# Anttwo/MACARONS

Hardware: AMD Instinct MI355X
Metric: candidate-camera coverage-gain evals/sec (100k pts, 200 cams) (higher is better)
Workload: dtype f32; 1 GPU; scorer: B=1 cloud x N=100000 points x C=200 cameras per GPU (BASELINE headline 100k pts / 200 cams), inputs resident in HBM; points=100000, cams_per_gpu=200, parallelism=camera-shard x1, streams=2

## Files before the change

macarons_amd/csrc/local_pct7.hip:

```cpp
#ifdef L7_TRACE
#define LP_TRACE L7_TRACE
#endif
#include "lp_tile.h"

namespace mcr {
namespace v7 {

using namespace tile;

#ifndef L7_PF
#define L7_PF 3
#endif
constexpr int PF = L7_PF;
__device__ __forceinline__ float l7_gelu(float x) {
    const float w = fabsf(x) * 0.84932180028801904f;
    const float t = __builtin_amdgcn_rcpf(fmaf(w, 0.39169198f, 1.0f));
    float q = fmaf(0.7478556f, t, -0.0958798f);
    q = fmaf(q, t, 0.3480242f);
    q *= t;
    const float e = __builtin_amdgcn_exp2f(-(w * w));
    const float erfa = fmaf(-q, e, 1.0f);
    const float hx = 0.5f * x;
    return fmaf(fabsf(hx), erfa, hx);
}

constexpr int PR = 17;
struct WRing { uint4 b[PF]; };

__device__ __forceinline__ const uint4* wptr(const float* Wp, int nt, int S, int lane) {
    return reinterpret_cast<const uint4*>(Wp) + (size_t)nt * S * 64 + lane;
}
template <int S>
__device__ __forceinline__ void wload(WRing& r, const uint4* bp) {
#pragma unroll
    for (int p = 0; p < (S < PF ? S : PF); ++p) {
        r.b[p] = bp[p * 64];
    }
    __builtin_amdgcn_sched_barrier(0);
}

__device__ __forceinline__ void fetch(uint4 (&an)[2], const uint4* __restrict__ A, int s, int i, int h) {
    const int c = 2 * s + h;
#pragma unroll
    for (int mt = 0; mt < 2; ++mt) an[mt] = A[(mt * 32 + i) * PR + c];
}

template <int S, class Fn>
__device__ __forceinline__ void gemm_with(f32x16 (&acc)[2], const uint4* __restrict__ A, WRing& r, const uint4* __restrict__ bp,
                                          int lane_, Fn fn) {
    const int lane = opaque(lane_);
    const int i = lane & 31, h = lane >> 5;
    uint4 an[2];
    fetch(an, A, 0, i, h);
#pragma unroll
    for (int s = 0; s < S; ++s) {
        const uint4 a0 = an[0], a1 = an[1];
        if (s + 1 < S) fetch(an, A, s + 1, i, h);
        const uint4 w = r.b[s % PF];
        if (s + PF < S) r.b[s % PF] = bp[(s + PF) * 64];
        __builtin_amdgcn_sched_barrier(0);
        acc[0] = mfma_h(w, a0, acc[0]);
        acc[1] = mfma_h(w, a1, acc[1]);
        fn(s);
        pin(acc[0], acc[1]);
        __builtin_amdgcn_sched_barrier(0);
    }
}
template <int S>
__device__ __forceinline__ void gemm(f32x16 (&acc)[2], const uint4* __restrict__ A, WRing& r, const uint4* __restrict__ bp,
                                     int lane_) {
    gemm_with<S>(acc, A, r, bp, lane_, [](int) {});
}

__device__ __forceinline__ void gemm_qkv(f32x16 (&acc)[2], f32x16& acch, const uint4* __restrict__ A, WRing& r0, WRing& r1,
                                         const uint4* __restrict__ bp0, const uint4* __restrict__ bp1, int wave, int lane_) {
    constexpr int S = 8;
    const int lane = opaque(lane_);
    const int i = lane & 31, h = lane >> 5, mh = wave & 1;
    uint4 an[2];
    fetch(an, A, 0, i, h);
#pragma unroll
    for (int s = 0; s < S; ++s) {
        const uint4 a0 = an[0], a1 = an[1];
        const uint4 ah = mh ? a1 : a0;
        if (s + 1 < S) fetch(an, A, s + 1, i, h);
        const uint4 w = r0.b[s % PF], v = r1.b[s % PF];
        if (s + PF < S) {
            r0.b[s % PF] = bp0[(s + PF) * 64];
            r1.b[s % PF] = bp1[(s + PF) * 64];
        }
        __builtin_amdgcn_sched_barrier(0);
        acc[0] = mfma_h(w, a0, acc[0]);
        acc[1] = mfma_h(w, a1, acc[1]);
        acch = mfma_h(v, ah, acch);
        pin(acc[0], acc[1], acch);
        __builtin_amdgcn_sched_barrier(0);
    }
}

__device__ __forceinline__ void add_bias(f32x16& x, const float* __restrict__ vec, int nt, int lane_) {
    const float4* p = reinterpret_cast<const float4*>(vec + 32 * nt + 4 * (opaque(lane_) >> 5));
#pragma unroll
    for (int g = 0; g < 4; ++g) {
        const float4 b = p[2 * g];
        x[4 * g] += b.x; x[4 * g + 1] += b.y; x[4 * g + 2] += b.z; x[4 * g + 3] += b.w;
    }
}

__device__ __forceinline__ void put4(uint2* __restrict__ plane, int idx, float v0, float v1, float v2, float v3) {
    plane[idx] = make_uint2(pack2h(v0, v1), pack2h(v2, v3));
}
template <class Fn>
__device__ __forceinline__ void put_planes(uint4* __restrict__ buf, int nt, int mt, const f32x16& t, int lane_, Fn f) {
    const int lane = opaque(lane_);
    const int j = lane & 31, h = lane >> 5;
    uint2* b2 = reinterpret_cast<uint2*>(buf) + (mt * 32 + j) * (2 * PR) + h + 8 * nt;
#pragma unroll
    for (int g = 0; g < 4; ++g) {
        put4(b2, 2 * g, f(t[4 * g], g, 0), f(t[4 * g + 1], g, 1), f(t[4 * g + 2], g, 2), f(t[4 * g + 3], g, 3));
        __builtin_amdgcn_sched_barrier(0);
    }
}
template <class Fn>
__device__ __forceinline__ void put_quad(uint4* __restrict__ buf, int nt, int mt, int g, const f32x16& t, int row, Fn f) {
    uint2* b2 = reinterpret_cast<uint2*>(buf);
    put4(b2, mt * (32 * 2 * PR) + row + 2 * (4 * nt + g), f(t[4 * g]), f(t[4 * g + 1]), f(t[4 * g + 2]), f(t[4 * g + 3]));
}
template <class Fn>
__device__ __forceinline__ void put_f32(float* __restrict__ buf, int LD, int kmask, int chunk0, int mt, const f32x16& t, int lane_, Fn f) {
    const int lane = opaque(lane_);
    const int j = lane & 31, h = lane >> 5, key = j & kmask;
    float* row = buf + (mt * 32 + j) * LD;
#pragma unroll
    for (int g = 0; g < 4; ++g)
        *reinterpret_cast<float4*>(row + (((chunk0 + 2 * g + h) ^ key) << 2)) =
            make_float4(f(t[4 * g], g, 0), f(t[4 * g + 1], g, 1), f(t[4 * g + 2], g, 2), f(t[4 * g + 3], g, 3));
}

__device__ __forceinline__ void ln_partial(const f32x16 (&x)[2], float2* __restrict__ St, int wave, int lane_) {
    const int lane = opaque(lane_);
#pragma unroll
    for (int mt = 0; mt < 2; ++mt) {
#ifdef L7_LN_TWO_PASS
        float s = 0.f;
#pragma unroll
        for (int r = 0; r < 16; r += 4) s += (x[mt][r] + x[mt][r + 1]) + (x[mt][r + 2] + x[mt][r + 3]);
        const float m = halves_sum(s) * (1.0f / 32.f);
        float q = 0.f;
#pragma unroll
        for (int r = 0; r < 16; ++r) {
            const float d = x[mt][r] - m;
            q = fmaf(d, d, q);
        }
        q = halves_sum(q);
        St[wave * 64 + mt * 32 + (lane & 31)] = make_float2(m, q);
#else
        float s = 0.f, q = 0.f;
#pragma unroll
        for (int r = 0; r < 16; r += 4) s += (x[mt][r] + x[mt][r + 1]) + (x[mt][r + 2] + x[mt][r + 3]);
#pragma unroll
        for (int r = 0; r < 16; ++r) q = fmaf(x[mt][r], x[mt][r], q);
        s = halves_sum(s);
        q = halves_sum(q);
        const float m = s * (1.0f / 32.f);
        St[wave * 64 + mt * 32 + (lane & 31)] = make_float2(m, fmaxf(fmaf(-s, m, q), 0.f));
#endif
    }
}
__device__ __forceinline__ void ln_finish(const f32x16 (&x)[2], const float2* __restrict__ St, uint4* __restrict__ P, int wave,
                                          int lane_) {
    const int j = opaque(lane_) & 31;
#pragma unroll
    for (int mt = 0; mt < 2; ++mt) {
        float2 p[4];
#pragma unroll
        for (int w = 0; w < 4; ++w) p[w] = St[w * 64 + mt * 32 + j];
        const float mu = ((p[0].x + p[1].x) + (p[2].x + p[3].x)) * 0.25f;
        float m2 = (p[0].y + p[1].y) + (p[2].y + p[3].y), dd = 0.f;
#pragma unroll
        for (int w = 0; w < 4; ++w) {
            const float d = p[w].x - mu;
            dd = fmaf(d, d, dd);
        }
        m2 = fmaf(32.f, dd, m2);
        const float rstd = __builtin_amdgcn_rsqf(fmaf(m2, 1.0f / 128.f, 1e-5f));
        const float shift = -mu * rstd;
        put_planes(P, wave, mt, x[mt], lane_, [&](float v, int, int) { return fmaf(v, rstd, shift); });
    }
}

#ifndef L7_WGS
#define L7_WGS 3
#endif
__global__ __launch_bounds__(256, L7_WGS) void local_pct7_kernel(const float* __restrict__ offs, float* __restrict__ feat,
                                                                long long ld_feat, long long S,
                                                                const float* __restrict__ blob, _Float16* __restrict__ feat_h) {
    __shared__ __attribute__((aligned(16))) uint4 P[64 * PR];
    __shared__ __attribute__((aligned(16))) uint4 H[2 * 64 * 16];
    __shared__ __attribute__((aligned(16))) float2 St[4 * 64];
    __shared__ __attribute__((aligned(16))) uint4 Z[4];
    float* F = reinterpret_cast<float*>(H);
    const int tid = threadIdx.x, lane0 = tid & 63;
    const int wave = __builtin_amdgcn_readfirstlane(tid >> 6);
    if (tid < 4) Z[tid] = make_uint4(0, 0, 0, 0);
    const float* mats = blob;
    const float* vecs = blob + L7_MATS_TOTAL;
    const long long s0 = (long long)blockIdx.x * L3_QPB;
    const int lane = lane0;
    int tp = 0; (void)tp;
    LP_T();
    WRing ring;
    f32x16 acc[2], xres[2];
    wload<1>(ring, wptr(mats + l7_mat_off(0), wave, 1, lane));
    init_bias(acc[0], vecs + LP_VEC_EMB1, wave, lane);
    init_bias(acc[1], vecs + LP_VEC_EMB1, wave, lane);
    float xyz[2][3];
    {
        const int j = lane & 31;
#pragma unroll
        for (int mt = 0; mt < 2; ++mt) {
            const int t = mt * 32 + j;
            const long long seq = s0 + (t >> 4);
            xyz[mt][0] = xyz[mt][1] = xyz[mt][2] = 0.f;
            if (seq < S) {
                const float* p = offs + (seq * 16 + (t & 15)) * 3;
                xyz[mt][0] = p[0]; xyz[mt][1] = p[1]; xyz[mt][2] = p[2];
            }
        }
        const bool lowh = lane < 32;
#pragma unroll
        for (int mt = 0; mt < 2; ++mt) {
            uint4 a = make_uint4(0, 0, 0, 0);
            a.x = pack2h(lowh ? xyz[mt][0] : 0.f, lowh ? xyz[mt][1] : 0.f);
            a.y = pack2h(lowh ? xyz[mt][2] : 0.f, 0.f);
            acc[mt] = mfma_h(ring.b[0], a, acc[mt]);
        }
    }
    LP_T();
    wload<8>(ring, wptr(mats + l7_mat_off(1), wave, 8, lane));
#pragma unroll
    for (int mt = 0; mt < 2; ++mt)
        put_planes(H, wave, mt, acc[mt], lane, [&](float v, int, int) { return l7_gelu(v); });
    init_bias(xres[0], vecs + LP_VEC_EMB2, wave, lane);
    init_bias(xres[1], vecs + LP_VEC_EMB2, wave, lane);
    __syncthreads();
    LP_T();
    gemm<8>(xres, H, ring, wptr(mats + l7_mat_off(1), wave, 8, lane), lane);
    LP_T();
    {
        const bool cat = wave == 3 && lane >= 32;
#pragma unroll
        for (int mt = 0; mt < 2; ++mt) {
            xres[mt][13] = cat ? xyz[mt][0] : xres[mt][13];
            xres[mt][14] = cat ? xyz[mt][1] : xres[mt][14];
            xres[mt][15] = cat ? xyz[mt][2] : xres[mt][15];
        }
    }

#pragma unroll 1
    for (int e = 0; e < 2; ++e) {
        const float* em = mats + l7_mat_off(2) + e * (L7_MAT_QKV + 5 * L7_MAT_128);
        const float* ev = vecs + LP_VEC_ENC0 + e * LP_VEC_ENC_STRIDE;
        const float* w_out = em + L7_MAT_QKV;
        const float* w_ff1a = w_out + L7_MAT_128;
        const float* w_ff1b = w_out + L7_MAT_128 * 2;
        const float* w_ff2a = w_out + L7_MAT_128 * 3;
        const float* w_ff2b = w_out + L7_MAT_128 * 4;
        WRing ring1;
        const uint4* bq0 = wptr(em, wave, 8, lane);
        const uint4* bq1 = wptr(em, 4 + (wave >> 1), 8, lane);
        wload<8>(ring, bq0);
        wload<8>(ring1, bq1);
        LP_T();
        ln_partial(xres, St, wave, lane);
        __syncthreads();
        LP_T();
        ln_finish(xres, St, P, wave, lane);
        __syncthreads();
        LP_T();
        {
            f32x16 aq[2], ah;
            const int nth = 4 + (wave >> 1);
            init_bias(aq[0], ev, wave, lane);
            init_bias(aq[1], ev, wave, lane);
            init_bias(ah, ev, nth, lane);
            gemm_qkv(aq, ah, P, ring, ring1, bq0, bq1, wave, lane);
            LP_T();
            wload<8>(ring, wptr(w_out, wave, 8, lane));
            __syncthreads();
            LP_T();
            auto fb = [&](float v, int, int) { return v; };
            uint4* dst = wave < 2 ? P : H;
            const int ntd = wave < 2 ? wave : wave - 2;
#pragma unroll
            for (int mt = 0; mt < 2; ++mt) put_planes(dst, ntd, mt, aq[mt], lane, fb);
            put_planes(H, nth - 2, wave & 1, ah, lane, fb);
        }
        __syncthreads();
        LP_T();
        {
            typedef _Float16 h16x4 __attribute__((ext_vector_type(4)));
            typedef short s16x4 __attribute__((ext_vector_type(4)));
            typedef __attribute__((address_space(3))) s16x4 lds_s16x4;
            const int ln = opaque(lane);
            const int r0 = wave * 16, li = ln & 15, g = ln >> 4;
            const char* Pb = reinterpret_cast<const char*>(P);
            const char* ka = Pb + (r0 + li) * (16 * PR) + 64 + (g & 1) * 8;
            const char* qa = g < 2 ? Pb + (r0 + li) * (16 * PR) + g * 8 : reinterpret_cast<const char*>(Z);
            const char* va = reinterpret_cast<const char*>(H) + (r0 + 4 * g + (li >> 2)) * (16 * PR) + (li & 3) * 8;
            h16x4 pf[4];
#pragma unroll
            for (int hh = 0; hh < 4; ++hh) {
                const h16x4 kf = *reinterpret_cast<const h16x4*>(ka + 16 * hh);
                const h16x4 qf = *reinterpret_cast<const h16x4*>(qa + 16 * hh);
                f32x4 st = __builtin_amdgcn_mfma_f32_16x16x16f16(kf, qf, f32x4{0.f, 0.f, 0.f, 0.f}, 0, 0, 0);
                float mx = fmaxf(fmaxf(st[0], st[1]), fmaxf(st[2], st[3]));
                mx = rows_allreduce(mx, [](float a, float b) { return fmaxf(a, b); });
                mx *= 0.35355339059327376220f;
                float den = 0.f;
#pragma unroll
                for (int r = 0; r < 4; ++r) {
                    st[r] = __expf(fmaf(st[r], 0.35355339059327376220f, -mx));
                    den += st[r];
                }
                den = rows_allreduce(den, [](float a, float b) { return a + b; });
                const float inv = __builtin_amdgcn_rcpf(den);
                const uint2 pk = make_uint2(pack2h(st[0] * inv, st[1] * inv), pack2h(st[2] * inv, st[3] * inv));
                pf[hh] = __builtin_bit_cast(h16x4, pk);
            }
            f32x4 o[4][2];
#pragma unroll
            for (int hh = 0; hh < 4; ++hh)
#pragma unroll
                for (int nt = 0; nt < 2; ++nt) {
                    const s16x4 vt = __builtin_amdgcn_ds_read_tr16_b64_v4i16((lds_s16x4*)(va + 64 * hh + 32 * nt));
                    o[hh][nt] = __builtin_amdgcn_mfma_f32_16x16x16f16(__builtin_bit_cast(h16x4, vt), pf[hh], f32x4{0.f, 0.f, 0.f, 0.f}, 0, 0, 0);
                }
            asm volatile("s_waitcnt lgkmcnt(0)" ::: "memory");
            uint2* p2 = reinterpret_cast<uint2*>(P);
            const int base = (r0 + li) * (2 * PR) + g;
#pragma unroll
            for (int hh = 0; hh < 4; ++hh)
#pragma unroll
                for (int nt = 0; nt < 2; ++nt)
                    put4(p2, base + 2 * (4 * hh + 2 * nt), o[hh][nt][0], o[hh][nt][1], o[hh][nt][2], o[hh][nt][3]);
        }
        LP_T();
        add_bias(xres[0], ev + 192, wave, lane);
        add_bias(xres[1], ev + 192, wave, lane);
        __syncthreads();
        LP_T();
        gemm<8>(xres, P, ring, wptr(w_out, wave, 8, lane), lane);
        LP_T();
        wload<8>(ring, wptr(w_ff1a, wave, 8, lane));
        ln_partial(xres, St, wave, lane);
        init_bias(acc[0], ev + 192 + 128, wave, lane);
        init_bias(acc[1], ev + 192 + 128, wave, lane);
        __syncthreads();
        LP_T();
        ln_finish(xres, St, P, wave, lane);
        __syncthreads();
        LP_T();
        gemm<8>(acc, P, ring, wptr(w_ff1a, wave, 8, lane), lane);
        LP_T();
        wload<8>(ring, wptr(w_ff1b, wave, 8, lane));
        f32x16 accb[2];
        init_bias(accb[0], ev + 192 + 128 + 128, wave, lane);
        init_bias(accb[1], ev + 192 + 128 + 128, wave, lane);
        const int pq_lane = opaque(lane), pq_row = (pq_lane & 31) * (2 * PR) + (pq_lane >> 5);
        gemm_with<8>(accb, P, ring, wptr(w_ff1b, wave, 8, lane), lane, [&](int s_) {
            put_quad(H, wave, s_ >> 2, s_ & 3, acc[s_ >> 2], pq_row, [&](float v) { return l7_gelu(v); });
        });
        LP_T();
        wload<8>(ring, wptr(w_ff2a, wave, 8, lane));
        add_bias(xres[0], ev + 192 + 128 + 256, wave, lane);
        add_bias(xres[1], ev + 192 + 128 + 256, wave, lane);
        __syncthreads();
        LP_T();
        gemm_with<8>(xres, H, ring, wptr(w_ff2a, wave, 8, lane), lane, [&](int s_) {
            put_quad(P, wave, s_ >> 2, s_ & 3, accb[s_ >> 2], pq_row, [&](float v) { return l7_gelu(v); });
        });
        LP_T();
        wload<8>(ring, wptr(w_ff2b, wave, 8, lane));
        __syncthreads();
        LP_T();
        LP_T();
        gemm<8>(xres, P, ring, wptr(w_ff2b, wave, 8, lane), lane);
        LP_T();
    }
    LP_T();
    wload<8>(ring, wptr(mats + l7_mat_off(14), wave, 8, lane));
    ln_partial(xres, St, wave, lane);
    init_bias(acc[0], vecs + LP_VEC_LIN0, wave, lane);
    init_bias(acc[1], vecs + LP_VEC_LIN0, wave, lane);
    __syncthreads();
    ln_finish(xres, St, P, wave, lane);
    __syncthreads();
    gemm<8>(acc, P, ring, wptr(mats + l7_mat_off(14), wave, 8, lane), lane);
#pragma unroll
    for (int mt = 0; mt < 2; ++mt)
        put_f32(F, 128, 15, 8 * wave, mt, acc[mt], lane, [&](float v, int, int) { return v; });
    __syncthreads();
    LP_T();
#pragma unroll
    for (int r = 0; r < 2; ++r) {
        const int o = tid + r * 256, q = o >> 7, c = o & 127;
        if (s0 + q < S) {
            float mx = -__builtin_inff(), sm = 0.f;
#pragma unroll
            for (int j = 0; j < 16; ++j) {
                const int row = q * 16 + j;
                const float v = F[row * 128 + ((((c >> 2) ^ (row & 15)) << 2) | (c & 3))];
                mx = fmaxf(mx, v);
                sm += v;
            }
            const float av = sm * (1.0f / 16.f);
            if (feat_h) {
                const unsigned hv = pack2h(mx, av);
                const long long o2 = (s0 + q) * ld_feat + c;
                feat_h[o2] = __builtin_bit_cast(_Float16, (unsigned short)(hv & 0xffffu));
                feat_h[o2 + 128] = __builtin_bit_cast(_Float16, (unsigned short)(hv >> 16));
            } else {
                feat[(s0 + q) * ld_feat + c] = mx;
                feat[(s0 + q) * ld_feat + 128 + c] = av;
            }
        }
    }
    LP_T();
}

}

void launch_local_pct7(hipStream_t s, const float* offs, float* feat, int64_t ld_feat, int64_t S, const float* blob, void* feat_h) {
    if (S <= 0) return;
    hipLaunchKernelGGL(v7::local_pct7_kernel, dim3((unsigned)cdiv(S, L3_QPB)), dim3(256), 0, s, offs, feat, (long long)ld_feat,
                       (long long)S, blob, (_Float16*)feat_h);
}

int local_pct7_blob_floats() { return L7_BLOB_FLOATS; }

}
```

Baseline: 4.777 million evals/s.

## Use logistic-form GELU fit, packed f16 mix FMAs, and precomputed lane byte offsets

Replaces the erf-polynomial GELU with a fitted logistic form x/(1+exp2(x*p(x^2))), using constants generated by a new minimax-fit script. LayerNorm normalisation and softmax scaling now write f16 pairs directly through v_fma_mix instructions, and the softmax uses exp2 with the log2(e) factor folded into the scale. Per-lane address components (weight, bias, fragment row, plane row, stats) are computed once into a Lane struct as byte offsets, which removes repeated index arithmetic and opaque() calls. The goal is fewer VALU instructions in the per-point MLP/attention kernel, at the cost of a slightly different GELU approximation error.

```diff
diff --git a/macarons_amd/csrc/gelu7_consts.inc b/macarons_amd/csrc/gelu7_consts.inc
--- /dev/null
+++ b/macarons_amd/csrc/gelu7_consts.inc
@@ -0,0 +1,4 @@
+constexpr float GELU7_K1 = -2.30112134f;
+constexpr float GELU7_K3 = -0.106775724f;
+constexpr float GELU7_K5 = 0.00101426308f;
+constexpr float GELU7_U0 = 64.0f;
diff --git a/macarons_amd/csrc/gen_gelu7_consts.py b/macarons_amd/csrc/gen_gelu7_consts.py
--- /dev/null
+++ b/macarons_amd/csrc/gen_gelu7_consts.py
@@ -0,0 +1,78 @@
+#!/usr/bin/env python3
+import math
+
+import numpy as np
+
+X = np.arange(-9000, 9001) * 1e-3
+PHI = np.array([0.5 * math.erfc(-x / math.sqrt(2.0)) for x in X])
+GELU = X * PHI
+U = X * X
+
+
+def max_err(c):
+    z = -X * (c[0] + U * (c[1] + U * c[2]))
+    with np.errstate(over="ignore"):
+        return float(np.max(np.abs(X / (1.0 + np.exp(z)) - GELU)))
+
+
+def nelder_mead(f, x0, step, iters=4000):
+    n = len(x0)
+    pts = [np.array(x0, dtype=np.float64)] + [np.array(x0, dtype=np.float64) + step[i] * np.eye(n)[i] for i in range(n)]
+    val = [f(p) for p in pts]
+    for _ in range(iters):
+        order = np.argsort(val)
+        pts, val = [pts[i] for i in order], [val[i] for i in order]
+        cen = np.mean(pts[:-1], axis=0)
+        refl = cen + (cen - pts[-1])
+        fr = f(refl)
+        if fr < val[0]:
+            ex = cen + 2.0 * (cen - pts[-1])
+            fe = f(ex)
+            pts[-1], val[-1] = (ex, fe) if fe < fr else (refl, fr)
+        elif fr < val[-2]:
+            pts[-1], val[-1] = refl, fr
+        else:
+            con = cen + 0.5 * (pts[-1] - cen)
+            fc = f(con)
+            if fc < val[-1]:
+                pts[-1], val[-1] = con, fc
+            else:
+                pts = [pts[0]] + [pts[0] + 0.5 * (p - pts[0]) for p in pts[1:]]
+                val = [val[0]] + [f(p) for p in pts[1:]]
+    k = int(np.argmin(val))
+    return pts[k], val[k]
+
+
+def fit():
+    sel = (X > 0) & (X <= 5.0)
+    x, ph = X[sel], PHI[sel]
+    y = np.log(ph / (1.0 - ph)) / x
+    A = np.stack([np.ones_like(x), x * x, x ** 4], axis=1)
+    c = np.linalg.lstsq(A, y, rcond=None)[0]
+    best = max_err(c)
+    for _ in range(12):
+        c2, e2 = nelder_mead(max_err, c, [1e-3 * abs(v) for v in c])
+        if e2 >= best * (1.0 - 1e-6):
+            break
+        c, best = c2, e2
+    return c, best
+
+
+def main():
+    c, err = fit()
+    u_star = -c[1] / (2.0 * c[2])
+    U0 = 64.0
+    p_u0 = c[0] + U0 * (c[1] + U0 * c[2])
+    assert c[2] < 0 and u_star < U0 and p_u0 > 1.0, (c, u_star, p_u0)
+    k = [-v / math.log(2.0) for v in c]
+    print("// Generated by gen_gelu7_consts.py -- do not edit.  Logistic-form erf GELU: x / (1 + exp(-x (c1 + c3 u + c5 u^2))), u = min(x^2, U0).")
+    print(f"// minimax fit on [-9, 9]: c = ({c[0]:.9g}, {c[1]:.9g}, {c[2]:.9g}), max |error| on the GELU {err:.3g} (double precision);")
+    print(f"// the polynomial peaks at u = {u_star:.4g} < U0; p(U0) = {p_u0:.4g}.  K = -log2(e) c: the exponent of v_exp_f32 directly.")
+    print(f"constexpr float GELU7_K1 = {k[0]:.9g}f;")
+    print(f"constexpr float GELU7_K3 = {k[1]:.9g}f;")
+    print(f"constexpr float GELU7_K5 = {k[2]:.9g}f;")
+    print(f"constexpr float GELU7_U0 = {U0:.1f}f;")
+
+
+if __name__ == "__main__":
+    main()
diff --git a/macarons_amd/csrc/local_pct7.hip b/macarons_amd/csrc/local_pct7.hip
--- a/macarons_amd/csrc/local_pct7.hip
+++ b/macarons_amd/csrc/local_pct7.hip
@@ -12,52 +12,73 @@
 #define L7_PF 3
 #endif
 constexpr int PF = L7_PF;
-__device__ __forceinline__ float l7_gelu(float x) {
-    const float w = fabsf(x) * 0.84932180028801904f;
-    const float t = __builtin_amdgcn_rcpf(fmaf(w, 0.39169198f, 1.0f));
-    float q = fmaf(0.7478556f, t, -0.0958798f);
-    q = fmaf(q, t, 0.3480242f);
-    q *= t;
-    const float e = __builtin_amdgcn_exp2f(-(w * w));
-    const float erfa = fmaf(-q, e, 1.0f);
-    const float hx = 0.5f * x;
-    return fmaf(fabsf(hx), erfa, hx);
-}
+#include "gelu7_consts.inc"
+__device__ __forceinline__ float l7_gate(float x) {
+    const float u = fminf(x * x, GELU7_U0);
+    float p = fmaf(u, GELU7_K5, GELU7_K3);
+    p = fmaf(p, u, GELU7_K1);
+    const float e = __builtin_amdgcn_exp2f(p * x);
+    return __builtin_amdgcn_rcpf(1.0f + e);
+}
+__device__ __forceinline__ unsigned fma2h(float a0, float b0, float c0, float a1, float b1, float c1) {
+    unsigned d;
+    asm("v_fma_mixlo_f16 %0, %1, %2, %3" : "=v"(d) : "v"(a0), "v"(b0), "v"(c0));
+    asm("v_fma_mixhi_f16 %0, %1, %2, %3" : "+v"(d) : "v"(a1), "v"(b1), "v"(c1));
+    return d;
+}
+__device__ __forceinline__ unsigned mul2h(float a0, float b0, float a1, float b1) {
+    unsigned d;
+    const float nz = -0.0f;
+    asm("v_fma_mixlo_f16 %0, %1, %2, %3" : "=v"(d) : "v"(a0), "v"(b0), "s"(nz));
+    asm("v_fma_mixhi_f16 %0, %1, %2, %3" : "+v"(d) : "v"(a1), "v"(b1), "s"(nz));
+    return d;
+}
+__device__ __forceinline__ unsigned gelu2h(float a, float b) { return mul2h(a, l7_gate(a), b, l7_gate(b)); }
 
 constexpr int PR = 17;
+constexpr int ROWB = 16 * PR;
 struct WRing { uint4 b[PF]; };
 
-__device__ __forceinline__ const uint4* wptr(const float* Wp, int nt, int S, int lane) {
-    return reinterpret_cast<const uint4*>(Wp) + (size_t)nt * S * 64 + lane;
+struct Lane {
+    unsigned w16;
+    unsigned b16;
+    unsigned frow;
+    unsigned prow;
+    unsigned st8;
+};
+
+__device__ __forceinline__ const char* wptr(const float* Wp, int nt, int S) {
+    return reinterpret_cast<const char*>(Wp) + (unsigned)(nt * S) * 1024u;
+}
+__device__ __forceinline__ uint4 wstep(const char* bp, int s, unsigned w16) {
+    return *reinterpret_cast<const uint4*>(bp + s * 1024 + w16);
 }
 template <int S>
-__device__ __forceinline__ void wload(WRing& r, const uint4* bp) {
+__device__ __forceinline__ void wload(WRing& r, const char* bp, unsigned w16) {
 #pragma unroll
     for (int p = 0; p < (S < PF ? S : PF); ++p) {
-        r.b[p] = bp[p * 64];
+        r.b[p] = wstep(bp, p, w16);
     }
     __builtin_amdgcn_sched_barrier(0);
 }
 
-__device__ __forceinline__ void fetch(uint4 (&an)[2], const uint4* __restrict__ A, int s, int i, int h) {
-    const int c = 2 * s + h;
-#pragma unroll
-    for (int mt = 0; mt < 2; ++mt) an[mt] = A[(mt * 32 + i) * PR + c];
+__device__ __forceinline__ void fetch(uint4 (&an)[2], const uint4* __restrict__ A, int s, unsigned frow) {
+    const char* a = reinterpret_cast<const char*>(A) + frow;
+#pragma unroll
+    for (int mt = 0; mt < 2; ++mt) an[mt] = *reinterpret_cast<const uint4*>(a + mt * 32 * ROWB + s * 32);
 }
 
 template <int S, class Fn>
-__device__ __forceinline__ void gemm_with(f32x16 (&acc)[2], const uint4* __restrict__ A, WRing& r, const uint4* __restrict__ bp,
-                                          int lane_, Fn fn) {
-    const int lane = opaque(lane_);
-    const int i = lane & 31, h = lane >> 5;
+__device__ __forceinline__ void gemm_with(f32x16 (&acc)[2], const uint4* __restrict__ A, WRing& r, const char* __restrict__ bp,
+                                          const Lane& L, Fn fn) {
     uint4 an[2];
-    fetch(an, A, 0, i, h);
+    fetch(an, A, 0, L.frow);
 #pragma unroll
     for (int s = 0; s < S; ++s) {
         const uint4 a0 = an[0], a1 = an[1];
-        if (s + 1 < S) fetch(an, A, s + 1, i, h);
+        if (s + 1 < S) fetch(an, A, s + 1, L.frow);
         const uint4 w = r.b[s % PF];
-        if (s + PF < S) r.b[s % PF] = bp[(s + PF) * 64];
+        if (s + PF < S) r.b[s % PF] = wstep(bp, s + PF, L.w16);
         __builtin_amdgcn_sched_barrier(0);
         acc[0] = mfma_h(w, a0, acc[0]);
         acc[1] = mfma_h(w, a1, acc[1]);
@@ -67,27 +88,26 @@
     }
 }
 template <int S>
-__device__ __forceinline__ void gemm(f32x16 (&acc)[2], const uint4* __restrict__ A, WRing& r, const uint4* __restrict__ bp,
-                                     int lane_) {
-    gemm_with<S>(acc, A, r, bp, lane_, [](int) {});
+__device__ __forceinline__ void gemm(f32x16 (&acc)[2], const uint4* __restrict__ A, WRing& r, const char* __restrict__ bp,
+                                     const Lane& L) {
+    gemm_with<S>(acc, A, r, bp, L, [](int) {});
 }
 
 __device__ __forceinline__ void gemm_qkv(f32x16 (&acc)[2], f32x16& acch, const uint4* __restrict__ A, WRing& r0, WRing& r1,
-                                         const uint4* __restrict__ bp0, const uint4* __restrict__ bp1, int wave, int lane_) {
+                                         const char* __restrict__ bp0, const char* __restrict__ bp1, int wave, const Lane& L) {
     constexpr int S = 8;
-    const int lane = opaque(lane_);
-    const int i = lane & 31, h = lane >> 5, mh = wave & 1;
+    const int mh = wave & 1;
     uint4 an[2];
-    fetch(an, A, 0, i, h);
+    fetch(an, A, 0, L.frow);
 #pragma unroll
     for (int s = 0; s < S; ++s) {
         const uint4 a0 = an[0], a1 = an[1];
         const uint4 ah = mh ? a1 : a0;
-        if (s + 1 < S) fetch(an, A, s + 1, i, h);
+        if (s + 1 < S) fetch(an, A, s + 1, L.frow);
         const uint4 w = r0.b[s % PF], v = r1.b[s % PF];
         if (s + PF < S) {
-            r0.b[s % PF] = bp0[(s + PF) * 64];
-            r1.b[s % PF] = bp1[(s + PF) * 64];
+            r0.b[s % PF] = wstep(bp0, s + PF, L.w16);
+            r1.b[s % PF] = wstep(bp1, s + PF, L.w16);
         }
         __builtin_amdgcn_sched_barrier(0);
         acc[0] = mfma_h(w, a0, acc[0]);
@@ -98,11 +118,20 @@
     }
 }
 
-__device__ __forceinline__ void add_bias(f32x16& x, const float* __restrict__ vec, int nt, int lane_) {
-    const float4* p = reinterpret_cast<const float4*>(vec + 32 * nt + 4 * (opaque(lane_) >> 5));
+__device__ __forceinline__ float4 bias4(const float* __restrict__ vec, int g, unsigned b16) {
+    return *reinterpret_cast<const float4*>(reinterpret_cast<const char*>(vec) + 32 * g + b16);
+}
+__device__ __forceinline__ void set_bias(f32x16& a, const float* __restrict__ vec, unsigned b16) {
 #pragma unroll
     for (int g = 0; g < 4; ++g) {
-        const float4 b = p[2 * g];
+        const float4 b = bias4(vec, g, b16);
+        a[4 * g] = b.x; a[4 * g + 1] = b.y; a[4 * g + 2] = b.z; a[4 * g + 3] = b.w;
+    }
+}
+__device__ __forceinline__ void add_bias(f32x16& x, const float* __restrict__ vec, unsigned b16) {
+#pragma unroll
+    for (int g = 0; g < 4; ++g) {
+        const float4 b = bias4(vec, g, b16);
         x[4 * g] += b.x; x[4 * g + 1] += b.y; x[4 * g + 2] += b.z; x[4 * g + 3] += b.w;
     }
 }
@@ -110,21 +139,18 @@
 __device__ __forceinline__ void put4(uint2* __restrict__ plane, int idx, float v0, float v1, float v2, float v3) {
     plane[idx] = make_uint2(pack2h(v0, v1), pack2h(v2, v3));
 }
-template <class Fn>
-__device__ __forceinline__ void put_planes(uint4* __restrict__ buf, int nt, int mt, const f32x16& t, int lane_, Fn f) {
-    const int lane = opaque(lane_);
-    const int j = lane & 31, h = lane >> 5;
-    uint2* b2 = reinterpret_cast<uint2*>(buf) + (mt * 32 + j) * (2 * PR) + h + 8 * nt;
+template <class Fn2>
+__device__ __forceinline__ void put_quad(uint4* __restrict__ buf, int mt, int g, const f32x16& t, unsigned row, Fn2 f2) {
+    *reinterpret_cast<uint2*>(reinterpret_cast<char*>(buf) + row + mt * 32 * ROWB + g * 16) =
+        make_uint2(f2(t[4 * g], t[4 * g + 1]), f2(t[4 * g + 2], t[4 * g + 3]));
+}
+template <class Fn2>
+__device__ __forceinline__ void put_planes(uint4* __restrict__ buf, int mt, const f32x16& t, unsigned row, Fn2 f2) {
 #pragma unroll
     for (int g = 0; g < 4; ++g) {
-        put4(b2, 2 * g, f(t[4 * g], g, 0), f(t[4 * g + 1], g, 1), f(t[4 * g + 2], g, 2), f(t[4 * g + 3], g, 3));
+        put_quad(buf, mt, g, t, row, f2);
         __builtin_amdgcn_sched_barrier(0);
     }
-}
-template <class Fn>
-__device__ __forceinline__ void put_quad(uint4* __restrict__ buf, int nt, int mt, int g, const f32x16& t, int row, Fn f) {
-    uint2* b2 = reinterpret_cast<uint2*>(buf);
-    put4(b2, mt * (32 * 2 * PR) + row + 2 * (4 * nt + g), f(t[4 * g]), f(t[4 * g + 1]), f(t[4 * g + 2]), f(t[4 * g + 3]));
 }
 template <class Fn>
 __device__ __forceinline__ void put_f32(float* __restrict__ buf, int LD, int kmask, int chunk0, int mt, const f32x16& t, int lane_, Fn f) {
@@ -137,8 +163,8 @@
             make_float4(f(t[4 * g], g, 0), f(t[4 * g + 1], g, 1), f(t[4 * g + 2], g, 2), f(t[4 * g + 3], g, 3));
 }
 
-__device__ __forceinline__ void ln_partial(const f32x16 (&x)[2], float2* __restrict__ St, int wave, int lane_) {
-    const int lane = opaque(lane_);
+__device__ __forceinline__ void ln_partial(const f32x16 (&x)[2], float2* __restrict__ St, int wave, const Lane& L) {
+    char* stw = reinterpret_cast<char*>(St + wave * 64) + L.st8;
 #pragma unroll
     for (int mt = 0; mt < 2; ++mt) {
 #ifdef L7_LN_TWO_PASS
@@ -153,7 +179,7 @@
             q = fmaf(d, d, q);
         }
         q = halves_sum(q);
-        St[wave * 64 + mt * 32 + (lane & 31)] = make_float2(m, q);
+        *reinterpret_cast<float2*>(stw + mt * 256) = make_float2(m, q);
 #else
         float s = 0.f, q = 0.f;
 #pragma unroll
@@ -163,18 +189,17 @@
         s = halves_sum(s);
         q = halves_sum(q);
         const float m = s * (1.0f / 32.f);
-        St[wave * 64 + mt * 32 + (lane & 31)] = make_float2(m, fmaxf(fmaf(-s, m, q), 0.f));
+        *reinterpret_cast<float2*>(stw + mt * 256) = make_float2(m, fmaxf(fmaf(-s, m, q), 0.f));
 #endif
     }
 }
-__device__ __forceinline__ void ln_finish(const f32x16 (&x)[2], const float2* __restrict__ St, uint4* __restrict__ P, int wave,
-                                          int lane_) {
-    const int j = opaque(lane_) & 31;
+__device__ __forceinline__ void ln_finish(const f32x16 (&x)[2], const float2* __restrict__ St, uint4* __restrict__ P, const Lane& L) {
+    const char* stj = reinterpret_cast<const char*>(St) + L.st8;
 #pragma unroll
     for (int mt = 0; mt < 2; ++mt) {
         float2 p[4];
 #pragma unroll
-        for (int w = 0; w < 4; ++w) p[w] = St[w * 64 + mt * 32 + j];
+        for (int w = 0; w < 4; ++w) p[w] = *reinterpret_cast<const float2*>(stj + w * 512 + mt * 256);
         const float mu = ((p[0].x + p[1].x) + (p[2].x + p[3].x)) * 0.25f;
         float m2 = (p[0].y + p[1].y) + (p[2].y + p[3].y), dd = 0.f;
 #pragma unroll
@@ -185,7 +210,7 @@
         m2 = fmaf(32.f, dd, m2);
         const float rstd = __builtin_amdgcn_rsqf(fmaf(m2, 1.0f / 128.f, 1e-5f));
         const float shift = -mu * rstd;
-        put_planes(P, wave, mt, x[mt], lane_, [&](float v, int, int) { return fmaf(v, rstd, shift); });
+        put_planes(P, mt, x[mt], L.prow, [&](float a, float b) { return fma2h(a, rstd, shift, b, rstd, shift); });
     }
 }
 
@@ -207,13 +232,20 @@
     const float* vecs = blob + L7_MATS_TOTAL;
     const long long s0 = (long long)blockIdx.x * L3_QPB;
     const int lane = lane0;
+    Lane L;
+    L.w16 = (unsigned)lane * 16u;
+    L.b16 = (unsigned)(lane >> 5) * 16u;
+    L.frow = (unsigned)(lane & 31) * ROWB + (unsigned)(lane >> 5) * 16u;
+    L.prow = (unsigned)(lane & 31) * ROWB + (unsigned)(lane >> 5) * 8u + (unsigned)wave * 64u;
+    L.st8 = (unsigned)(lane & 31) * 8u;
+    const int wv32 = wave * 32;
     int tp = 0; (void)tp;
     LP_T();
     WRing ring;
     f32x16 acc[2], xres[2];
-    wload<1>(ring, wptr(mats + l7_mat_off(0), wave, 1, lane));
-    init_bias(acc[0], vecs + LP_VEC_EMB1, wave, lane);
-    init_bias(acc[1], vecs + LP_VEC_EMB1, wave, lane);
+    wload<1>(ring, wptr(mats + l7_mat_off(0), wave, 1), L.w16);
+    set_bias(acc[0], vecs + LP_VEC_EMB1 + wv32, L.b16);
+    set_bias(acc[1], vecs + LP_VEC_EMB1 + wv32, L.b16);
     float xyz[2][3];
     {
         const int j = lane & 31;
@@ -237,15 +269,15 @@
         }
     }
     LP_T();
-    wload<8>(ring, wptr(mats + l7_mat_off(1), wave, 8, lane));
+    wload<8>(ring, wptr(mats + l7_mat_off(1), wave, 8), L.w16);
 #pragma unroll
     for (int mt = 0; mt < 2; ++mt)
-        put_planes(H, wave, mt, acc[mt], lane, [&](float v, int, int) { return l7_gelu(v); });
-    init_bias(xres[0], vecs + LP_VEC_EMB2, wave, lane);
-    init_bias(xres[1], vecs + LP_VEC_EMB2, wave, lane);
+        put_planes(H, mt, acc[mt], L.prow, [](float a, float b) { return gelu2h(a, b); });
+    set_bias(xres[0], vecs + LP_VEC_EMB2 + wv32, L.b16);
+    set_bias(xres[1], vecs + LP_VEC_EMB2 + wv32, L.b16);
     __syncthreads();
     LP_T();
-    gemm<8>(xres, H, ring, wptr(mats + l7_mat_off(1), wave, 8, lane), lane);
+    gemm<8>(xres, H, ring, wptr(mats + l7_mat_off(1), wave, 8), L);
     LP_T();
     {
         const bool cat = wave == 3 && lane >= 32;
@@ -267,34 +299,36 @@
         const float* w_ff2a = w_out + L7_MAT_128 * 3;
         const float* w_ff2b = w_out + L7_MAT_128 * 4;
         WRing ring1;
-        const uint4* bq0 = wptr(em, wave, 8, lane);
-        const uint4* bq1 = wptr(em, 4 + (wave >> 1), 8, lane);
-        wload<8>(ring, bq0);
-        wload<8>(ring1, bq1);
-        LP_T();
-        ln_partial(xres, St, wave, lane);
-        __syncthreads();
-        LP_T();
-        ln_finish(xres, St, P, wave, lane);
+        const char* bq0 = wptr(em, wave, 8);
+        const char* bq1 = wptr(em, 4 + (wave >> 1), 8);
+        wload<8>(ring, bq0, L.w16);
+        wload<8>(ring1, bq1, L.w16);
+        LP_T();
+        ln_partial(xres, St, wave, L);
+        __syncthreads();
+        LP_T();
+        ln_finish(xres, St, P, L);
         __syncthreads();
         LP_T();
         {
             f32x16 aq[2], ah;
             const int nth = 4 + (wave >> 1);
-            init_bias(aq[0], ev, wave, lane);
-            init_bias(aq[1], ev, wave, lane);
-            init_bias(ah, ev, nth, lane);
-            gemm_qkv(aq, ah, P, ring, ring1, bq0, bq1, wave, lane);
+            set_bias(aq[0], ev + wv32, L.b16);
+            set_bias(aq[1], ev + wv32, L.b16);
+            set_bias(ah, ev + 32 * nth, L.b16);
+            gemm_qkv(aq, ah, P, ring, ring1, bq0, bq1, wave, L);
             LP_T();
-            wload<8>(ring, wptr(w_out, wave, 8, lane));
+            wload<8>(ring, wptr(w_out, wave, 8), L.w16);
             __syncthreads();
             LP_T();
-            auto fb = [&](float v, int, int) { return v; };
+            auto fb = [](float a, float b) { return pack2h(a, b); };
             uint4* dst = wave < 2 ? P : H;
             const int ntd = wave < 2 ? wave : wave - 2;
-#pragma unroll
-            for (int mt = 0; mt < 2; ++mt) put_planes(dst, ntd, mt, aq[mt], lane, fb);
-            put_planes(H, nth - 2, wave & 1, ah, lane, fb);
+            const unsigned rowq = L.prow + (unsigned)((ntd - wave) * 64);
+            const unsigned rowh = L.prow + (unsigned)((nth - 2 - wave) * 64 + (wave & 1) * (32 * ROWB));
+#pragma unroll
+            for (int mt = 0; mt < 2; ++mt) put_planes(dst, mt, aq[mt], rowq, fb);
+            put_planes(H, 0, ah, rowh, fb);
         }
         __syncthreads();
         LP_T();
@@ -316,16 +350,17 @@
                 f32x4 st = __builtin_amdgcn_mfma_f32_16x16x16f16(kf, qf, f32x4{0.f, 0.f, 0.f, 0.f}, 0, 0, 0);
                 float mx = fmaxf(fmaxf(st[0], st[1]), fmaxf(st[2], st[3]));
                 mx = rows_allreduce(mx, [](float a, float b) { return fmaxf(a, b); });
-                mx *= 0.35355339059327376220f;
+                constexpr float SC = 0.35355339059327376220f * 1.44269504088896340736f;
+                mx *= SC;
                 float den = 0.f;
 #pragma unroll
                 for (int r = 0; r < 4; ++r) {
-                    st[r] = __expf(fmaf(st[r], 0.35355339059327376220f, -mx));
+                    st[r] = __builtin_amdgcn_exp2f(fmaf(st[r], SC, -mx));
                     den += st[r];
                 }
                 den = rows_allreduce(den, [](float a, float b) { return a + b; });
                 const float inv = __builtin_amdgcn_rcpf(den);
-                const uint2 pk = make_uint2(pack2h(st[0] * inv, st[1] * inv), pack2h(st[2] * inv, st[3] * inv));
+                const uint2 pk = make_uint2(mul2h(st[0], inv, st[1], inv), mul2h(st[2], inv, st[3], inv));
                 pf[hh] = __builtin_bit_cast(h16x4, pk);
             }
             f32x4 o[4][2];
@@ -346,57 +381,56 @@
                     put4(p2, base + 2 * (4 * hh + 2 * nt), o[hh][nt][0], o[hh][nt][1], o[hh][nt][2], o[hh][nt][3]);
         }
         LP_T();
-        add_bias(xres[0], ev + 192, wave, lane);
-        add_bias(xres[1], ev + 192, wave, lane);
-        __syncthreads();
-        LP_T();
-        gemm<8>(xres, P, ring, wptr(w_out, wave, 8, lane), lane);
-        LP_T();
-        wload<8>(ring, wptr(w_ff1a, wave, 8, lane));
-        ln_partial(xres, St, wave, lane);
-        init_bias(acc[0], ev + 192 + 128, wave, lane);
-        init_bias(acc[1], ev + 192 + 128, wave, lane);
-        __syncthreads();
-        LP_T();
-        ln_finish(xres, St, P, wave, lane);
-        __syncthreads();
-        LP_T();
-        gemm<8>(acc, P, ring, wptr(w_ff1a, wave, 8, lane), lane);
-        LP_T();
-        wload<8>(ring, wptr(w_ff1b, wave, 8, lane));
+        add_bias(xres[0], ev + 192 + wv32, L.b16);
+        add_bias(xres[1], ev + 192 + wv32, L.b16);
+        __syncthreads();
+        LP_T();
+        gemm<8>(xres, P, ring, wptr(w_out, wave, 8), L);
+        LP_T();
+        wload<8>(ring, wptr(w_ff1a, wave, 8), L.w16);
+        ln_partial(xres, St, wave, L);
+        set_bias(acc[0], ev + 192 + 128 + wv32, L.b16);
+        set_bias(acc[1], ev + 192 + 128 + wv32, L.b16);
+        __syncthreads();
+        LP_T();
+        ln_finish(xres, St, P, L);
+        __syncthreads();
+        LP_T();
+        gemm<8>(acc, P, ring, wptr(w_ff1a, wave, 8), L);
+        LP_T();
+        wload<8>(ring, wptr(w_ff1b, wave, 8), L.w16);
         f32x16 accb[2];
-        init_bias(accb[0], ev + 192 + 128 + 128, wave, lane);
-        init_bias(accb[1], ev + 192 + 128 + 128, wave, lane);
-        const int pq_lane = opaque(lane), pq_row = (pq_lane & 31) * (2 * PR) + (pq_lane >> 5);
-        gemm_with<8>(accb, P, ring, wptr(w_ff1b, wave, 8, lane), lane, [&](int s_) {
-            put_quad(H, wave, s_ >> 2, s_ & 3, acc[s_ >> 2], pq_row, [&](float v) { return l7_gelu(v); });
+        set_bias(accb[0], ev + 192 + 128 + 128 + wv32, L.b16);
+        set_bias(accb[1], ev + 192 + 128 + 128 + wv32, L.b16);
+        gemm_with<8>(accb, P, ring, wptr(w_ff1b, wave, 8), L, [&](int s_) {
+            put_quad(H, s_ >> 2, s_ & 3, acc[s_ >> 2], L.prow, [](float a, float b) { return gelu2h(a, b); });
         });
         LP_T();
-        wload<8>(ring, wptr(w_ff2a, wave, 8, lane));
-        add_bias(xres[0], ev + 192 + 128 + 256, wave, lane);
-        add_bias(xres[1], ev + 192 + 128 + 256, wave, lane);
-        __syncthreads();
-        LP_T();
-        gemm_with<8>(xres, H, ring, wptr(w_ff2a, wave, 8, lane), lane, [&](int s_) {
-            put_quad(P, wave, s_ >> 2, s_ & 3, accb[s_ >> 2], pq_row, [&](float v) { return l7_gelu(v); });
+        wload<8>(ring, wptr(w_ff2a, wave, 8), L.w16);
+        add_bias(xres[0], ev + 192 + 128 + 256 + wv32, L.b16);
+        add_bias(xres[1], ev + 192 + 128 + 256 + wv32, L.b16);
+        __syncthreads();
+        LP_T();
+        gemm_with<8>(xres, H, ring, wptr(w_ff2a, wave, 8), L, [&](int s_) {
+            put_quad(P, s_ >> 2, s_ & 3, accb[s_ >> 2], L.prow, [](float a, float b) { return gelu2h(a, b); });
         });
         LP_T();
-        wload<8>(ring, wptr(w_ff2b, wave, 8, lane));
-        __syncthreads();
-        LP_T();
-        LP_T();
-        gemm<8>(xres, P, ring, wptr(w_ff2b, wave, 8, lane), lane);
-        LP_T();
-    }
-    LP_T();
-    wload<8>(ring, wptr(mats + l7_mat_off(14), wave, 8, lane));
-    ln_partial(xres, St, wave, lane);
-    init_bias(acc[0], vecs + LP_VEC_LIN0, wave, lane);
-    init_bias(acc[1], vecs + LP_VEC_LIN0, wave, lane);
+        wload<8>(ring, wptr(w_ff2b, wave, 8), L.w16);
+        __syncthreads();
+        LP_T();
+        LP_T();
+        gemm<8>(xres, P, ring, wptr(w_ff2b, wave, 8), L);
+        LP_T();
+    }
+    LP_T();
+    wload<8>(ring, wptr(mats + l7_mat_off(14), wave, 8), L.w16);
+    ln_partial(xres, St, wave, L);
+    set_bias(acc[0], vecs + LP_VEC_LIN0 + wv32, L.b16);
+    set_bias(acc[1], vecs + LP_VEC_LIN0 + wv32, L.b16);
     __syncthreads();
-    ln_finish(xres, St, P, wave, lane);
+    ln_finish(xres, St, P, L);
     __syncthreads();
-    gemm<8>(acc, P, ring, wptr(mats + l7_mat_off(14), wave, 8, lane), lane);
+    gemm<8>(acc, P, ring, wptr(mats + l7_mat_off(14), wave, 8), L);
 #pragma unroll
     for (int mt = 0; mt < 2; ++mt)
         put_f32(F, 128, 15, 8 * wave, mt, acc[mt], lane, [&](float v, int, int) { return v; });
```

After: 4.770 million evals/s. No clear change (-0.1%).
